# huangnengCSU/longcallR

Measured on AMD Instinct MI355X. Metric: candidate_sites_per_sec, higher is better.
Workload: dtype u8 in, u32 counts, f64 likelihoods, i64 fixed-point phase scores

## Files before the change

### include/lcr.h

```cpp
#ifndef LCR_H
#define LCR_H
#include <stddef.h>
#include <stdint.h>
#ifdef __cplusplus
extern "C" {
#endif

#define LCR_OK 0
#define LCR_E_ARG (-1)
#define LCR_E_CIGAR (-2)
#define LCR_E_DEVICE (-3)
#define LCR_E_STATE (-4)
#define LCR_E_NOMEM (-5)
#define LCR_W_HW_QUEUES 1

#define LCR_PLATFORM_HIFI 0
#define LCR_PLATFORM_ONT 1

#define LCR_MEM_HOST 0
#define LCR_MEM_DEVICE 1

typedef struct lcr_ctx lcr_ctx;


// ... 358 lines not shown
int lcr_debug_set(lcr_ctx*, const char* key, int64_t value);

enum { LCR_K_SPANS = 0 , LCR_K_PILEUP, LCR_K_CAND_FILTER, LCR_K_CAND_HIST, LCR_K_CAND_GT,
       LCR_K_FRAG_COUNT, LCR_K_FRAG_FILL, LCR_K_PHASE,
       LCR_K_BIND ,
       LCR_K_BIND_TABLE ,
       LCR_K_CAND_IMPORT , LCR_K_JUNCTIONS ,
       LCR_K_ASE , LCR_NKERNELS };
enum { LCR_K_GENES = LCR_NKERNELS ,
       LCR_K_ASE_GENES ,
       LCR_NTIMERS };
int lcr_enable_timing(lcr_ctx*, int on);
int lcr_kernel_ms(lcr_ctx*, int kernel, float* ms);
int lcr_pileup_bytes(lcr_ctx*, int64_t* bytes);
int lcr_pileup_stage_bytes(lcr_ctx*, int64_t* bytes);

int lcr_release_cached_memory(void);
int lcr_set_cache_limits(int64_t device_bytes, int64_t host_bytes);

const char* lcr_version(void);

#ifdef __cplusplus
}
#endif
#endif
```

### longcallr_amd/_lib.py

```python
import ctypes as C
import os

from . import _abi

_HERE = os.path.dirname(os.path.abspath(__file__))
SO_PATH = os.environ.get("LCR_LIB") or os.path.join(_HERE, "liblcr.so")

SYMBOLS = [
    "lcr_params_preset", "lcr_ctx_create", "lcr_ctx_destroy", "lcr_last_error", "lcr_ctx_set_stream",
    "lcr_ctx_sync", "lcr_ctx_set_lock_dir", "lcr_ctx_set_async_phase", "lcr_debug_set", "lcr_load_batch", "lcr_load_batch_async", "lcr_bind_batch",
    "lcr_host_alloc", "lcr_host_free", "lcr_host_register", "lcr_host_unregister", "lcr_pileup", "lcr_get_columns", "lcr_candidates",
    "lcr_get_candidates", "lcr_get_candidates_device", "lcr_fragments", "lcr_get_fragmat", "lcr_phase", "lcr_get_phase_result", "lcr_get_read_records_device", "lcr_collect_phase", "lcr_get_ld_blocks", "lcr_get_tie_census",
    "lcr_enable_timing", "lcr_kernel_ms", "lcr_pileup_bytes", "lcr_pileup_stage_bytes", "lcr_discover_regions", "lcr_discover_regions_truncated", "lcr_version", "lcr_release_cached_memory", "lcr_set_cache_limits",
    "lcr_bam_open", "lcr_bam_open_keep", "lcr_bam_close", "lcr_bam_last_error", "lcr_bam_refs", "lcr_bam_n_records", "lcr_bam_resident", "lcr_bam_spans", "lcr_bam_batch", "lcr_bam_write_phased", "lcr_bam_write_reads",
    "lcr_set_downsample", "lcr_set_downsample_rows", "lcr_get_downsample",
    "lcr_junctions", "lcr_get_junctions", "lcr_ase", "lcr_get_ase", "lcr_vcf_contig_alleles",
    "lcr_assign_genes", "lcr_get_read_genes", "lcr_ase_genes", "lcr_get_ase_genes",
    "lcr_junctions_genes", "lcr_get_junctions_genes", "lcr_asj_genes", "lcr_get_asj_genes",
    "lcr_load_batch_packed", "lcr_load_batch_packed_async", "lcr_unpack_bases", "lcr_unpack_ms", "lcr_bam_batch_packed",
    "lcr_set_exon_mask", "lcr_exon_mask_ms", "lcr_import_candidates", "lcr_vcf_open", "lcr_vcf_close", "lcr_vcf_last_error", "lcr_vcf_contigs", "lcr_vcf_contig",
    "lcr_haplotag", "lcr_get_haplotag_sites", "lcr_haplotag_ms", "lcr_vcf_contig_phase_sets",
    "lcr_site_counts", "lcr_get_site_counts", "lcr_site_counts_ms",
    "lcr_hap_coverage", "lcr_get_hap_coverage", "lcr_hap_coverage_ms",
    "lcr_somatic", "lcr_get_somatic", "lcr_somatic_ms",
]

_lib = None

# ... 47 lines not shown
    l.lcr_get_read_records_device.argtypes = [vp, C.POINTER(vp), C.POINTER(i32)]
    l.lcr_get_fragmat.argtypes = [vp, C.POINTER(_abi.LcrFragmat)]
    l.lcr_get_phase_result.argtypes = [vp, C.POINTER(_abi.LcrPhaseResult)]
    l.lcr_collect_phase.argtypes = [vp, C.POINTER(_abi.LcrPhaseCollected)]
    l.lcr_release_cached_memory.argtypes = []
    l.lcr_set_cache_limits.argtypes = [C.c_int64, C.c_int64]
    l.lcr_get_tie_census.argtypes = [vp, C.POINTER(C.c_uint64)]
    l.lcr_get_ld_blocks.argtypes = [vp, C.c_int32, C.POINTER(C.c_int32), C.POINTER(C.POINTER(C.c_int32)), C.POINTER(C.POINTER(C.c_int32))]
    l.lcr_discover_regions.argtypes = [vp, C.c_int32, C.c_int32, vp, vp, C.c_int64, C.POINTER(_abi.LcrRegionList)]
    l.lcr_discover_regions_truncated.argtypes = [vp, C.c_int32, C.c_int32, vp, vp, C.c_int64, C.c_int32, C.c_uint32, C.POINTER(_abi.LcrRegionList),
                                                 C.POINTER(C.c_int64)]
    l.lcr_enable_timing.argtypes = [vp, i32]
    l.lcr_kernel_ms.argtypes = [vp, i32, C.POINTER(C.c_float)]
    l.lcr_pileup_bytes.argtypes = [vp, C.POINTER(C.c_int64)]
    l.lcr_pileup_stage_bytes.argtypes = [vp, C.POINTER(C.c_int64)]
    flt = C.POINTER(_abi.LcrReadFilter)
    l.lcr_bam_open.argtypes = [C.c_char_p, C.c_int32, C.POINTER(vp)]
    l.lcr_bam_open_keep.argtypes = [C.c_char_p, C.c_int32, C.c_int64, C.POINTER(vp)]
    l.lcr_bam_close.argtypes = [vp]
    l.lcr_bam_close.restype = None
    l.lcr_bam_last_error.argtypes = [vp]
    l.lcr_bam_last_error.restype = C.c_char_p
    l.lcr_bam_refs.argtypes = [vp, C.POINTER(C.c_int32), C.POINTER(C.POINTER(C.c_char_p)), C.POINTER(C.POINTER(C.c_int64))]
    l.lcr_bam_n_records.argtypes = [vp, C.POINTER(C.c_int64)]
    l.lcr_bam_resident.argtypes = [vp, C.POINTER(C.c_int64), C.POINTER(C.c_int64)]
    l.lcr_bam_spans.argtypes = [vp, C.c_int32, flt, C.POINTER(C.c_int32), C.POINTER(C.POINTER(C.c_int32)), C.POINTER(C.POINTER(C.c_int32))]
    l.lcr_bam_batch.argtypes = [vp, C.c_int32, flt, C.c_int32, vp, vp, C.POINTER(_abi.LcrReads), C.POINTER(C.POINTER(C.c_int32)),
                                C.POINTER(C.POINTER(C.c_uint64)), C.POINTER(C.c_char_p)]
    l.lcr_bam_batch_packed.argtypes = [vp, C.c_int32, flt, C.c_int32, vp, vp, C.POINTER(_abi.LcrReadsPacked), C.POINTER(C.POINTER(C.c_int32)),
                                       C.POINTER(C.POINTER(C.c_uint64)), C.POINTER(C.c_char_p)]
# ... 44 lines not shown
```

### longcallr_amd/api.py

```python
import ctypes as C

import numpy as np

from . import _abi, _lib
from ._lib import LcrError


def _view(ptr, dtype, n):
    if n == 0 or not ptr:
        return np.zeros(0, dtype=dtype)
    buf = (C.c_char * (np.dtype(dtype).itemsize * n)).from_address(ptr)
    return np.frombuffer(buf, dtype=dtype, count=n).copy()


def _view_nocopy(ptr, dtype, n):
    if n == 0 or not ptr:
        return np.zeros(0, dtype=dtype)
    buf = (C.c_char * (np.dtype(dtype).itemsize * n)).from_address(ptr)
    return np.frombuffer(buf, dtype=dtype, count=n)


_DEBUG_ENV = {"LCR_PHASE_PROF": "phase_prof", "LCR_GRID_MIN_ENTRIES": "grid_min_entries",
              "LCR_GRID_GENERIC": "grid_generic", "LCR_GRID_SPEC_LANES": "grid_spec_lanes", "LCR_GRID_SPEC_BATCH": "grid_spec_batch", "LCR_POST_HALF": "post_half", "LCR_ENUM_FORCE_BIG": "enum_force_big",
              "LCR_ENUM_FORCE_STREAM": "enum_force_stream", "LCR_ENUM_ELIDE": "enum_elide", "LCR_HIST_TILES": "hist_tiles", "LCR_TIE_ARITH": "tie_arith", "LCR_CHAIN_TIES": "chain_ties", "LCR_K3_HITS": "k3_hits", "LCR_K3_LIST_BLOCKS": "k3_list_blocks", "LCR_FUSE_FILTER": "fuse_filter", "LCR_ASYNC_PHASE": "async_phase", "LCR_HOST_TRACE": "host_trace", "LCR_OWN_FILL": "own_fill", "LCR_REDO_LDS": "redo_lds", "LCR_SPEC_COMPACT": "spec_compact", "LCR_LEAN_PLANES": "lean_planes"}


class Engine:
    def __init__(self, device=0, params=None, timing=False):
        self.lib = _lib.load()
        h = C.c_void_p()
        rc = self.lib.lcr_ctx_create(device, C.byref(h))
        if rc != 0:
            raise LcrError("lcr_ctx_create(device=%d) failed with %d: no usable HIP device; "
                           "liblcr has no CPU fallback" % (device, rc))
        self.h = h
        self.device = device
        self.params = params if params is not None else _abi.make_params()
        self._sites = None
        self._keep = None
# ... 456 lines not shown
    def kernel_ms(self, k):
        ms = C.c_float()
        self._chk(self.lib.lcr_kernel_ms(self.h, k, C.byref(ms)), "lcr_kernel_ms")
        return float(ms.value)

    def pileup_bytes(self):
        b = C.c_int64()
        self._chk(self.lib.lcr_pileup_bytes(self.h, C.byref(b)), "lcr_pileup_bytes")
        return int(b.value)

    def pileup_stage_bytes(self):
        b = C.c_int64()
        self._chk(self.lib.lcr_pileup_stage_bytes(self.h, C.byref(b)), "lcr_pileup_stage_bytes")
        return int(b.value)


def host_register(*arrays):
    lib = _lib.load()
    done = []
    for a in arrays:
        if a is None or a.nbytes == 0:
            continue
        if lib.lcr_host_register(C.c_void_p(a.ctypes.data), a.nbytes) != 0:
            host_unregister(done)
            raise LcrError("lcr_host_register failed")
        done.append(a)
    return done


def host_unregister(arrays):
# ... 4 lines not shown
```

### longcallr_amd/csrc/k0_ops.hip

```cpp
#include <algorithm>
#include <climits>

#include "lcr_dev.h"

#ifndef K0_THREADS
#define K0_THREADS 256
#endif
#ifndef K0_OPT
#define K0_OPT 4
#endif
#ifndef K0_ABL
#define K0_ABL 0
#endif
#define K0_NW (K0_THREADS / 64)
#define K0_WIN K0_THREADS
#define K0_ACC 64
#ifndef K0_HCAP
#define K0_HCAP 160
#endif


__device__ __forceinline__ int wave_incl_max(int v) {
  v = max(v, __builtin_amdgcn_update_dpp(0, v, 0x111, 0xf, 0xf, false));
  v = max(v, __builtin_amdgcn_update_dpp(0, v, 0x112, 0xf, 0xf, false));
// ... 56 lines not shown
  uint64_t seq_off;
  int32_t reb, rel_pos;
};

__device__ __forceinline__ void wave_lds_sync() {
  __builtin_amdgcn_fence(__ATOMIC_RELEASE, "wavefront");
  __builtin_amdgcn_wave_barrier();
  __builtin_amdgcn_fence(__ATOMIC_ACQUIRE, "wavefront");
}

template <int OPT>
__global__ void __launch_bounds__(K0_THREADS)
k0_ops(BatchView b, const ReadBin* __restrict__ rbin, const int32_t* __restrict__ blk_first_read, uint64_t cig0, uint32_t n_ops,
       int ont, int D, int32_t n_tiles, int32_t* __restrict__ tile_fill, int32_t* __restrict__ tile_nchunks, int32_t* __restrict__ tile_ndiff,
       K0Ctl* __restrict__ ctl, unsigned int* __restrict__ acct, unsigned int pool_sub, unsigned long long* __restrict__ recs,
       unsigned int desc_sub, uint32_t* __restrict__ desc_tile, uint2* __restrict__ desc_val, int2* __restrict__ read_scan) {
  constexpr int OPB = OPT * K0_THREADS, WOPS = OPT * 64;
  __shared__ __attribute__((aligned(8))) uint16_t ridh[OPB];
  __shared__ K0Hdr hdr[K0_HCAP];
  __shared__ int ws_ref[K0_NW], ws_q[K0_NW], ws_rid[K0_NW];
  __shared__ int cnt[K0_WIN], cur[K0_WIN];
  __shared__ unsigned int s_base[3];
  __shared__ int runbase[OPB];
  __shared__ int s_carry[2], s_acc[2];

  const int tid = threadIdx.x, lane = tid & 63, wv = tid >> 6;
  const uint32_t j0 = blockIdx.x * (uint32_t)OPB;
  if (j0 >= n_ops) return;
  const uint32_t jend = min(j0 + (uint32_t)OPB, n_ops);
  const bool last_block = jend == n_ops;
  const uint32_t* __restrict__ cg = b.cigar + cig0;
// ... 88 lines not shown
#pragma unroll
    for (int k = 0; k < OPT; k++) {
      xr[k] += br; xq[k] += bq; rid[k] = max(rid[k], bm);
      if (mark[k] != 0) {
        if (mark[k] < K0_HCAP) { hdr[mark[k]].refbase -= xr[k]; hdr[mark[k]].qbase -= xq[k]; }
        else read_scan[r_lo + mark[k]] = make_int2(xr[k], xq[k]);
      }
    }
    if (tid == 0) { hdr[0].refbase += s_carry[0]; hdr[0].qbase += s_carry[1]; }
  }
  __syncthreads();

  if (K0_ABL == 2) { if (xr[0] + xq[1] + rid[2] == 0x7fffffff) ctl->error = 9; return; }
  int a[OPT], e[OPT], tb[OPT], kind[OPT];
  unsigned int rlo[OPT], rhi[OPT];
  unsigned int my_items = 0;
  const int win0 = hdr[0].ftile + (int)((unsigned int)max(hdr[0].rel_pos - 1, 0) / (unsigned int)LCR_TILE);
#pragma unroll
  for (int k = 0; k < OPT; k++) {
    const int p = OPT * tid + k;
    const bool act = j0 + p < jend;
    K0Hdr H;
    if (rid[k] < K0_HCAP) H = hdr[rid[k]];
    else {
      uint64_t cb; int ncig;
      H = load_hdr(r_lo + rid[k], &cb, &ncig);
      const int2 sb = read_scan[r_lo + rid[k]];
      H.refbase -= sb.x; H.qbase -= sb.y;
    }
    const int op = w[k] & 15, len = (int)(w[k] >> 4);
    const int rs = H.refbase + xr[k];
    const int qs = H.qbase + xq[k];
    const bool m = act && (op == 0 || op == 7 || op == 8), d = act && op == 2, ins = act && op == 1, isn = act && op == 3;
    int aa = max(rs, 0), ee = min(rs + len, H.vec);
    if (m) { aa = max(aa, rs + (H.qlo - qs)); ee = min(ee, rs + (H.qhi - qs)); }
    int kd = ((m || d || isn) && len > 0 && ee > aa) ? (m ? 1 : d ? 2 : 4) : 0;
    if (ins && len > 0 && rs >= 1 && rs < H.vec) { kd = 3; aa = rs - 1; ee = rs; }
    kind[k] = kd; a[k] = aa; e[k] = ee; tb[k] = H.ftile;
    if (kd == 1) {
      const unsigned long long o0 = H.seq_off + (unsigned long long)(long long)(qs - rs);
      rlo[k] = (unsigned int)o0; rhi[k] = ((unsigned int)(o0 >> 32) & 0xffu) | H.hi;
    } else {
      rlo[k] = kd == 2 ? (unsigned int)REC_KIND_D : kd == 3 ? (unsigned int)REC_KIND_I : (unsigned int)REC_KIND_N;
      rhi[k] = 0xffu;
    }
    if (kd) my_items++;
    if (act && p == H.cend - 1) {
      b.read_rend[r_lo + rid[k]] = rs + dr[k];
      if (qs + dq[k] != H.reb) atomicExch(&ctl->error, 2);
    }
    if (kd == 4) {
      const int ta = H.ftile + (int)((unsigned int)aa / (unsigned int)LCR_TILE), te = H.ftile + (int)((unsigned int)(ee - 1) / (unsigned int)LCR_TILE);
      if (te > ta + 1) { atomicAdd(&tile_ndiff[ta + 1], 1); atomicAdd(&tile_ndiff[te], -1); }
    }
  }

  if (K0_ABL == 3) { int x = 0; for (int k = 0; k < OPT; k++) x += a[k] + e[k] + tb[k] + kind[k] + (int)rlo[k] + (int)rhi[k]; if (x == 0x7fffffff) ctl->error = 9; return; }
  auto make_rec = [&](int k, int t) -> unsigned long long {
    const int c0 = (t - tb[k]) * LCR_TILE;
    const int c_lo = max(a[k], c0), c_hi = min(e[k], c0 + LCR_TILE);
    unsigned int lo = rlo[k], hi = rhi[k] | ((unsigned int)(c_lo - c0) << 8) | ((unsigned int)(c_hi - c_lo - 1) << 18);
    if (kind[k] == 1) {
      const unsigned int s = lo + (unsigned int)c_lo;
      hi = (hi & ~0xffu) | (((hi & 0xffu) + (s < lo ? 1u : 0u)) & 0xffu);
      lo = s;
    }
    return ((unsigned long long)hi << 32) | lo;
  };
  auto first_tile = [&](int k) { return tb[k] + (int)((unsigned int)a[k] / (unsigned int)LCR_TILE); };
  auto last_tile = [&](int k) { return tb[k] + (int)((unsigned int)(e[k] - 1) / (unsigned int)LCR_TILE); };
  auto next_tile = [&](int k, int t, int te) { return kind[k] == 4 ? te : t + 1; };

  int key[OPT], rank[OPT], hpos[OPT];
  bool is_last[OPT];
  {
#pragma unroll
    for (int k = 0; k < OPT; k++) {
      const int tp = kind[k] ? first_tile(k) - win0 : -1;
      key[k] = (tp >= 0 && tp < K0_WIN) ? tp : -1;
    }
    int pk = __shfl_up(key[OPT - 1], 1, 64);
    if (lane == 0) pk = -2;
    bool head[OPT];
    int hp = 0;
#pragma unroll
    for (int k = 0; k < OPT; k++) {
      head[k] = key[k] != (k == 0 ? pk : key[k - 1]);
      if (head[k]) hp = OPT * lane + k + 1;
      hpos[k] = hp;
    }
    const int ih = wave_incl_max(hp);
    int bh = __shfl_up(ih, 1, 64);
    if (lane == 0) bh = 0;
    const int nh = __shfl_down(head[0] ? 1 : 0, 1, 64);
#pragma unroll
    for (int k = 0; k < OPT; k++) {
      hpos[k] = max(hpos[k], bh) - 1;
      rank[k] = OPT * lane + k - hpos[k];
      is_last[k] = k + 1 < OPT ? head[k + 1] : (lane == 63 || nh != 0);
      if (is_last[k] && key[k] >= 0) atomicAdd(&cnt[key[k]], rank[k] + 1);
      if (kind[k]) {
        const int te = last_tile(k);
        for (int t = first_tile(k); t < te;) {
          t = next_tile(k, t, te);
          const int wi = t - win0;
          if (wi >= 0 && wi < K0_WIN) atomicAdd(&cnt[wi], 1);
        }
      }
    }
  }
  __syncthreads();

  if (K0_ABL == 4) { int x = 0; for (int k = 0; k < OPT; k++) x += rank[k] + hpos[k] + (is_last[k] ? 1 : 0); if (x == 0x7fffffff) ctl->error = 9; return; }
  unsigned int my_recs = 0;
  const unsigned int shard = blockIdx.x % K0_ACC;
  {
// ... 21 lines not shown
    if (c > 0 && s_base[2]) {
      const int tile = win0 + tid;
      const unsigned int di = s_base[1] + (unsigned int)dbefore + (unsigned int)__popcll(nzb & ((1ull << lane) - 1ull));
      desc_tile[di] = (uint32_t)tile; desc_val[di] = make_uint2(s_base[0] + (unsigned int)(before + ic - c16), (unsigned int)c);
      atomicAdd(&tile_fill[tile], c);
      atomicAdd(&tile_nchunks[tile], c16 >> 4);
    }
  }
  const unsigned int blk_at = s_base[0];
  const bool blk_fits = s_base[2] != 0;

  auto put = [&](int slot, unsigned long long rec) { if (blk_fits) recs[blk_at + (unsigned int)slot] = rec; };
  int* rbw = runbase + wv * WOPS;
#pragma unroll
  for (int k = 0; k < OPT; k++)
    if (is_last[k] && key[k] >= 0) rbw[hpos[k]] = atomicAdd(&cur[key[k]], rank[k] + 1);
  wave_lds_sync();
  bool overflow = false;
#pragma unroll
  for (int k = 0; k < OPT; k++) {
    if (key[k] >= 0) put(rbw[hpos[k]] + rank[k], make_rec(k, first_tile(k)));
    else if (kind[k]) overflow = true;
    if (kind[k]) {
      const int te = last_tile(k);
      for (int t = first_tile(k); t < te;) {
        t = next_tile(k, t, te);
        const int wi = t - win0;
        if (wi >= 0 && wi < K0_WIN) put(atomicAdd(&cur[wi], 1), make_rec(k, t));
        else overflow = true;
      }
    }
  }
  if (overflow) {
#pragma unroll
    for (int k = 0; k < OPT; k++) {
      if (!kind[k]) continue;
      const int te = last_tile(k);
      for (int t = first_tile(k);; t = next_tile(k, t, te)) {
        if (t - win0 < 0 || t - win0 >= K0_WIN) {
          unsigned int* sh = acct + 32 * shard;
          const unsigned int at = atomicAdd(&sh[2], 1u), di = atomicAdd(&sh[3], 1u);
          if (at >= pool_sub || di >= desc_sub) atomicExch(&ctl->error, 3);
          else {
            recs[shard * pool_sub + at] = make_rec(k, t);
            desc_tile[shard * desc_sub + di] = (uint32_t)t; desc_val[shard * desc_sub + di] = make_uint2(shard * pool_sub + at, 1u);
            atomicAdd(&tile_fill[t], 1);
            atomicAdd(&tile_nchunks[t], 1);
          }
          my_recs++;
        }
        if (t >= te) break;
// ... 34 lines not shown
    const int ne = (int)((d.y + 15u) >> 4);
    uint2* dst = sorted + chunk_off[t] + atomicAdd(&cursor[t], ne);
    for (int e = 0; e < ne; e++) dst[e] = make_uint2(d.x + 16u * (unsigned int)e, min(16u, d.y - 16u * (unsigned int)e));
  }
}
void launch_k0_desc_bin(const K0Ctl* ctl, const unsigned int* acct, unsigned int desc_sub, const uint32_t* desc_tile, const void* desc_val,
                        const int32_t* chunk_off, int32_t* cursor, void* sorted, int32_t n_blocks_hint, hipStream_t s) {
  const int per = std::max(1, std::min((n_blocks_hint + K0_ACC - 1) / K0_ACC, 32));
  hipLaunchKernelGGL(k0_desc_bin, dim3(per * K0_ACC), dim3(LCR_BLOCK), 0, s, ctl, acct, desc_sub, desc_tile, (const uint2*)desc_val,
                     chunk_off, cursor, (uint2*)sorted);
}

void launch_k0_ops(const BatchView& b, const ReadBin* rb, const int32_t* blk_first_read, uint64_t cig0, uint32_t n_ops, int ont, int D,
                   int32_t n_tiles, int32_t* tile_fill, int32_t* tile_nchunks, int32_t* tile_ndiff, K0Ctl* ctl, unsigned int* acct,
                   unsigned int pool_sub, unsigned long long* recs, unsigned int desc_sub, uint32_t* desc_tile, void* desc_val, void* read_scan,
                   hipStream_t s) {
  if (b.n_reads == 0) return;
  if (n_ops == 0) { hipLaunchKernelGGL(k0_empty_reads, dim3((b.n_reads + LCR_BLOCK - 1) / LCR_BLOCK), dim3(LCR_BLOCK), 0, s, b, rb, ctl); return; }
  const int opb = launch_k0_opb();
  hipLaunchKernelGGL(k0_ops<K0_OPT>, dim3((n_ops + opb - 1) / opb), dim3(K0_THREADS), 0, s, b, rb, blk_first_read, cig0, n_ops, ont, D, n_tiles,
                     tile_fill, tile_nchunks, tile_ndiff, ctl, acct, pool_sub, recs, desc_sub, desc_tile, (uint2*)desc_val, (int2*)read_scan);
}
```

### longcallr_amd/csrc/k1_pileup.hip

```cpp
#include <algorithm>
#include <climits>

#include "lcr_dev.h"
#include "k2_eval.h"

#ifdef LCR_K1_ABLATE
#define K1_ABL LCR_K1_ABLATE
#else
#define K1_ABL 0
#endif
#ifndef K1_THREADS
#define K1_THREADS LCR_TILE
#endif
#define K1_WAVES (K1_THREADS / 64)
#define K1_CPT (LCR_TILE / K1_THREADS)
#define K1_RPB 2
#define K1_PMAP (8 * K1_THREADS)
#ifndef K1_NT_STORES
#define K1_NT_STORES 0
#endif
#ifndef K1_PIF
#define K1_PIF 4
#endif

// ... 244 lines not shown
  unsigned long long rec_nx[K1_RPB];
  int has_nx = load_recs(tid * K1_RPB, rec_nx);
  for (int rbase = 0; rbase < n_slots && K1_ABL != 3; rbase += K1_RPB * K1_THREADS) {
    unsigned long long rec_cur[K1_RPB];
#pragma unroll
    for (int x = 0; x < K1_RPB; x++) rec_cur[x] = rec_nx[x];
    const int has_cur = has_nx;
    has_nx = load_recs(rbase + K1_RPB * K1_THREADS + tid * K1_RPB, rec_nx);
    int npc[K1_RPB], nsum = 0;
#pragma unroll
    for (int x = 0; x < K1_RPB; x++) {
      const int slot = tid * K1_RPB + x;
      const unsigned long long rec = rec_cur[x];
      const bool hasrec = (has_cur >> x) & 1;
      const unsigned long long off = rec & REC_OFF_MASK;
      const int col0 = (int)((rec >> 40) & 1023u), len = (int)((rec >> 50) & 1023u) + 1;
      int npieces = 0;
      if (hasrec) {
        if (off == REC_KIND_D) {
          atomicAdd(&pl[P_DIFF_D * TSTRIDE + col0], 1u);
          atomicAdd(&pl[P_DIFF_D * TSTRIDE + col0 + len], 0xFFFFFFFFu);
        } else if (off == REC_KIND_I) {
          atomicAdd(&pl[P_NI * TSTRIDE + col0], 1u);
        } else if (off == REC_KIND_N) {
          atomicAdd(&pl[P_DIFF_N * TSTRIDE + col0], 1u);
          atomicAdd(&pl[P_DIFF_N * TSTRIDE + col0 + len], 0xFFFFFFFFu);
        } else {
          const int strand = (int)((rec >> 60) & 1u), tscls = (int)((rec >> 61) & 3u);
          uint32_t* dp = pl + (strand ? P_DIFF_DEPTH_R : P_DIFF_DEPTH_F) * TSTRIDE;
          atomicAdd(&dp[col0], 1u);
          atomicAdd(&dp[col0 + len], 0xFFFFFFFFu);
          if (tscls) {
            uint32_t* tp = pl + (tscls == 2 ? P_DIFF_TS1 : P_DIFF_TS0) * TSTRIDE;
            atomicAdd(&tp[col0], 1u);
            atomicAdd(&tp[col0 + len], 0xFFFFFFFFu);
          }
          npieces = (len + 15) >> 4;
        }
      }
      rec_s[slot] = rec;
      npc[x] = K1_ABL == 1 ? 0 : npieces;
      nsum += npc[x];
    }
    int run = block_incl_scan(nsum, wsum) - nsum;
    int P = 0;
#pragma unroll
    for (int i = 0; i < K1_WAVES; i++) P += wsum[i];
    const int pstride = (P + K1_PMAP - 1) / K1_PMAP;
    if (tid == 0) pstart[0] = 0;
#pragma unroll
    for (int x = 0; x < K1_RPB; x++) {
// ... 3 lines not shown
      if (pstride == 1) for (int q = first; q < run; q++) pown[q] = (uint16_t)(tid * K1_RPB + x);
      else if (pstride > 1) for (int k = (first + pstride - 1) / pstride; k * pstride < run; k++) pown[k] = (uint16_t)(tid * K1_RPB + x);
    }
    __syncthreads();
    struct Piece { uint4 v; int colA, k_lo, k_hi, strand; bool ok; };
    auto fetch = [&](int p) -> Piece {
      Piece q;
      q.ok = p < P;
      if (!q.ok) { q.v = make_uint4(0, 0, 0, 0); q.colA = 0; q.k_lo = q.k_hi = 0; q.strand = 0; return q; }
      int lo;
      if (pstride == 1) lo = pown[p];
      else { lo = pown[p / pstride]; while (pstart[lo + 1] <= p) lo++; }
      const unsigned long long rc = rec_s[lo];
      const uint32_t rhi = (uint32_t)(rc >> 32);
      const long long soff = (long long)(rc & REC_OFF_MASK);
      const int scol = (int)((rhi >> 8) & 1023u), slen = (int)((rhi >> 18) & 1023u) + 1;
      q.strand = (int)((rhi >> 28) & 1u);
      const int d16 = 16 * (p - pstart[lo]);
      const long long A = soff + d16;
      q.k_lo = 0; q.k_hi = min(16, slen - d16);
      q.colA = scol + d16;
      if (A + 16 <= b.n_bases) q.v = *reinterpret_cast<const uint4*>(b.bases + A);
      else {
        uint32_t t[4] = {0, 0, 0, 0};
        for (int x = 0; x < 16; x++)
          if (A + x < b.n_bases) t[x >> 2] |= (uint32_t)b.bases[A + x] << (8 * (x & 3));
        q.v = make_uint4(t[0], t[1], t[2], t[3]);
      }
      return q;
    };
    auto tally = [&](const Piece& q) {
// ... 567 lines not shown
```

### longcallr_amd/csrc/k2_candidates.hip

```cpp
#include "lcr_dev.h"
#include "k2_eval.h"

#define SCAN_ITEMS 4
#define SCAN_TILE (LCR_BLOCK * SCAN_ITEMS)

__device__ __forceinline__ int wave_incl_scan_i(int v, int lane) {
#pragma unroll
  for (int d = 1; d < 64; d <<= 1) {
    int t = __shfl_up(v, d, 64);
    if (lane >= d) v += t;
  }
  return v;
}
__device__ __forceinline__ long long wave_incl_scan_ll(long long v, int lane) {
#pragma unroll
  for (int d = 1; d < 64; d <<= 1) {
    long long t = __shfl_up(v, d, 64);
    if (lane >= d) v += t;
  }
  return v;
}

template <typename OutT>
__global__ void __launch_bounds__(LCR_BLOCK) scan_phase1(const int32_t* __restrict__ in, OutT* __restrict__ out, int32_t n,
// ... 295 lines not shown
    for (int i = tid; i < pc; i += HT_BLOCK) slot_of[sv[s0 + p0 + i].col - tc0] = (uint16_t)i;
    __syncthreads();
    const int c_lo = sv[s0 + p0].col - tc0, c_hi = sv[s0 + p0 + pc - 1].col - tc0;
    auto fetch = [&](int j) -> unsigned long long {
      if (j >= j_hi) return ~0ull;
      const uint2 en = ents[e0 + (j >> 4)];
      return ((unsigned int)j & 15u) < en.y ? recs[en.x + ((unsigned int)j & 15u)] : ~0ull;
    };
    unsigned long long nx = fetch(j_lo + grp), nx2 = fetch(j_lo + grp + HT_BLOCK / HT_LANES);
    for (int j = j_lo + grp; j < j_hi; j += HT_BLOCK / HT_LANES) {
      const unsigned long long rec = nx;
      nx = nx2;
      nx2 = fetch(j + 2 * (HT_BLOCK / HT_LANES));
      const unsigned long long off = rec & REC_OFF_MASK;
      const bool live = off < REC_KIND_N;
      const int col0 = (int)((rec >> 40) & 1023u), len = (int)((rec >> 50) & 1023u) + 1;
      const int d_lo = max(0, c_lo - col0), d_hi = live ? min(len - 1, c_hi - col0) : -1;
      auto tally = [&](int dd, bool in, uint32_t base, uint32_t qual) {
        const uint32_t slot = slot_of[min(col0 + max(dd, 0), LCR_TILE - 1)];
        const uint32_t u = (base & 0xDFu) - 65u;
        const bool acgt = u < 20u && ((0x80045u >> u) & 1u);
        const uint32_t k = ((base & 0xDFu) >> 1) & 3u, bi = k ^ (k >> 1);
        const uint32_t q = min(qual, 30u);
        const uint32_t idx = slot * 124u + bi * 31u + q;
        if (in && acgt && slot != 0xFFFFu) atomicAdd(&hp[idx >> 1], 1u << (16 * (idx & 1u)));
      };
      for (int d0 = d_lo + 4 * ln; d0 <= d_hi; d0 += 4 * HT_LANES) {
        const unsigned long long at = off + (unsigned long long)d0;
        uint32_t bw, qw;
        if (at + 4 <= (unsigned long long)b.n_bases) {
          bw = *reinterpret_cast<const uint32_t*>(b.bases + at); qw = *reinterpret_cast<const uint32_t*>(b.quals + at);
// ... 267 lines not shown
```

### longcallr_amd/csrc/lcr_api.hip

```cpp
#include <chrono>
#include <cmath>
#include <cstdlib>
#include <map>
#include <mutex>

#include "lcr_ctx.h"

namespace {
struct BlockCache {
  std::mutex mu;
  std::multimap<size_t, void*> blocks[2][16];
  size_t held[2][16] = {};
  size_t limit[2] = {(size_t)24 << 30, (size_t)2 << 30};
};
BlockCache& block_cache() { static BlockCache* c = new BlockCache(); return *c; }
}
void* lcr_cache_take(int host, size_t want, size_t* cap) {
  int dev = 0;
  if (hipGetDevice(&dev) != hipSuccess || dev < 0 || dev >= 16) return nullptr;
  BlockCache& bc = block_cache();
  std::lock_guard<std::mutex> g(bc.mu);
  auto& m = bc.blocks[host ? 1 : 0][dev];
  auto it = m.lower_bound(want);
  if (it == m.end() || it->first > 2 * want + (1u << 20)) return nullptr;
// ... 203 lines not shown

int lcr_pileup_bytes(lcr_ctx* c, int64_t* bytes) {
  if (!c || !bytes) return LCR_E_ARG;
  int64_t staged = 0;
  const int rc = pile_staged_bytes(c, &staged);
  *bytes = c->pileup_bytes + staged;
  return rc;
}

int lcr_pileup_stage_bytes(lcr_ctx* c, int64_t* bytes) {
  if (!c || !bytes) return LCR_E_ARG;
  int64_t staged = 0;
  const int rc = pile_staged_bytes(c, &staged);
  *bytes = c->stage_bytes + staged;
  return rc;
}

int lcr_phase(lcr_ctx* c, const lcr_params* p) {
  if (!c || !p) return LCR_E_ARG;
  if (c->stage < ST_FRAGGED) { c->err = "lcr_phase before lcr_fragments"; return LCR_E_STATE; }
  if (c->cand_used) { c->err = "lcr_phase after lcr_phase: the phase stage has rewritten the candidate records; run the candidate stage again"; return LCR_E_STATE; }
  if (p->ld_weight_threshold != 1) { c->err = "ld_weight_threshold must be 1: SNPFrag::phase is only ever called with 1 (thread.rs:166)"; return LCR_E_ARG; }
  const bool ds_on = c->ds_rows_set || c->ds_depth > 0;
  if (ds_on && !(p->read_assign_cutoff > 0.0)) { c->err = "down-sampling needs read_assign_cutoff > 0: the last read assignment must not depend on the sign of an unsampled row's haplotag"; return LCR_E_ARG; }
  HIPCHK(c, hipSetDevice(c->device));
  { int rc = frag_settle(c); if (rc) return rc; }
  PhaseInputs in;
  in.ds_depth = c->ds_depth; in.ds_seed = c->ds_seed; in.ds_rows = c->ds_rows_set ? c->ds_rows.data() : nullptr;
  c->ds_rows_set = false;
  in.n_regions = c->bv.n_regions; in.n_rows = c->n_rows; in.nnz = c->nnz;
// ... 230 lines not shown
        HIPCHK(c, hipMemcpyAsync(host.data(), buf.p, 4 * N, hipMemcpyDeviceToHost, c->stream));
        HIPCHK(c, hipStreamSynchronize(c->stream));
        if (host != want) { c->err = "fill_selftest: a fill kernel wrote other bytes than asked (offset " + std::to_string(off) + ", length " + std::to_string(len) + ")"; return LCR_E_DEVICE; }
      }
  }
  else if (k == "chain_ties") d.chain_ties = value != 0;
  else if (k == "redo_lds") d.redo_lds = (int)std::max<int64_t>(0, std::min<int64_t>(value, 128 * 1024));
  else if (k == "tie_arith") d.tie_arith = (int)std::max<int64_t>(0, std::min<int64_t>(value, 3));
  else if (k == "timing_mask") c->timing_mask = (uint32_t)value;
  else if (k == "hist_tiles") c->dbg_hist_tiles = value > 0 ? 1 : value < 0 ? -1 : 0;
  else if (k == "k3_hits") c->dbg_k3_hits = value != 0;
  else if (k == "k3_list_blocks") c->dbg_k3_list_blocks = (int)std::max<int64_t>(0, std::min<int64_t>(value, 65536));
  else if (k == "fuse_filter") c->dbg_fuse_filter = value != 0;
  else if (k == "spec_compact") c->dbg_spec_compact = value != 0;
  else if (k == "lean_planes") c->dbg_lean_planes = value != 0;
  else if (k == "poison_planes") c->dbg_poison_planes = value != 0;
  else if (k == "grid_spec_batch") d.spec_batch = (int)value;
  else if (k == "grid_spec_lanes") d.spec_lanes = (int)std::max<int64_t>(1, std::min<int64_t>(value, 16));
  else { c->err = "lcr_debug_set: unknown key " + k; return LCR_E_ARG; }
  return LCR_OK;
}

int lcr_get_ld_blocks(lcr_ctx* c, int32_t region, int32_t* n_blocks, const int32_t** block_off, const int32_t** snp_idx) {
  if (!c || !n_blocks || !block_off || !snp_idx) return LCR_E_ARG;
  if (c->stage < ST_PHASED) { c->err = "lcr_get_ld_blocks before lcr_phase"; return LCR_E_STATE; }
  if (region < 0 || region >= c->bv.n_regions) { c->err = "lcr_get_ld_blocks: no such region"; return LCR_E_ARG; }
  { int rc = phase_settle(c); if (rc) return rc; }
  PhaseInputs in;
  in.n_regions = c->bv.n_regions;
  in.cand_region_off = c->h_cand_off.data();
// ... 16 lines not shown
```

### longcallr_amd/csrc/lcr_ctx.h

```cpp
#pragma once
#include <algorithm>
#include <cstring>

#include "lcr_dev.h"
#include "lcr_phase_host.h"

enum Stage { ST_NONE, ST_LOADED, ST_PILED, ST_CALLED, ST_FRAGGED, ST_PHASED };

struct AnnotationCopy { DevBuf span_s, span_e, exon_off, exon_s, exon_e; };

struct SlotTable {
  int32_t n_slots = 0;
  DevBuf tbl_key, tbl_cnt, flag, koff;
  DevBuf ck, cc, cp;
  DevBuf off;
};

struct GeneJunctions {
  bool valid = false;
  bool timed = false;
  int32_t n = 0, ng = 0;
  AnnotationCopy ann;
  DevBuf part, nocc, part_off, occ_off, cnt, pair_off, read_pair, row_slot, pregion, pgene, prow0, prows, pocc, tsz, tbl_off, rows, keys, jpair;
  SlotTable t;
// ... 35 lines not shown
  struct UploadSlot { DevBuf buf[16]; DevBuf seq4, pack_off;
                      hipEvent_t ev = nullptr; bool filled = false; lcr_reads rd{}; lcr_regions rg{}; } up[2];
  hipStream_t up_stream = nullptr;
  int bound_slot = -1;
  bool bound_host = false;
  DevBuf in_seq4, in_pack_off, unpacked;
  HostBuf h_unpack_bad;
  hipEvent_t ev_unpack_t[2] = {};
  bool unpack_timed = false;
  DevBuf scan_tmp, read_region, read_bin, read_rend, tile_region, tile_col0, first_tile, k0_tile_fill, k0_items, tile_nbase, tile_order;
  DevBuf desc_tile, desc_val, chunks, chunk_off;
  DevBuf blk_first_read, read_scan, cig_compact, cig_off_new, cig_new_off32;
  uint64_t cig0 = 0;
  uint32_t n_ops = 0;
  int64_t n_items = 0;

  bool planes_dense = false;
  bool planes_tallied = false;
  int dbg_poison_planes = 0;
  int dbg_lean_planes = 1;
  DevBuf planes;
  bool sv_staged = false;
  int32_t sv_stage_cap = 0;
  int64_t sv_stage_n = -1;
  DevBuf sv_stage, sv_stage_key;
  DevParams dp{};
  int32_t pile_platform = -1; uint32_t pile_dist_to_end = 0;
  float sor_thr = -1.f;
  HostBuf h_planes;
  HostBuf h_nnz;
// ... 226 lines not shown
```

### longcallr_amd/csrc/lcr_dev.h

```cpp
#pragma once
#include <hip/hip_runtime.h>
#include <climits>
#include <cstddef>
#include <stdint.h>

#include <string>
#include <vector>

#include "../../include/lcr.h"

#ifndef LCR_TILE
#define LCR_TILE 256
#endif
#define LCR_BLOCK 256
#define LCR_WAVE 64

struct BatchView {
  int32_t n_reads, n_regions;
  int64_t n_bases;
  const int32_t* pos;
  const int32_t* seq_len;
  const int32_t* lead;
  const int32_t* trail;
  const uint8_t* flags;
// ... 26 lines not shown
  int32_t flags, pad_;
  int64_t pad2_;
};
static_assert(sizeof(ReadBin) == 64, "ReadBin must be 64 bytes");

struct DevParams {
  int32_t ont;
  int32_t dist_to_end, polya_len;
  uint32_t min_baseq, min_depth, max_depth, min_qual, low_cnt_cut, min_linkers;
  int32_t use_strand_bias;
  float min_af, min_af_intron, low_frac_cut;
  float sor_threshold;
  int32_t dbg;
};

#define REC_OFF_MASK 0xFFFFFFFFFFull
#define REC_KIND_D 0xFFFFFFFFFFull
#define REC_KIND_I 0xFFFFFFFFFEull
#define REC_KIND_N 0xFFFFFFFFFDull

struct Survivor {
  int64_t gcol;
  int32_t region;
  int32_t col;
  uint8_t ref_base, allele1, allele2, n_alt;
  uint32_t cnt1, cnt2, depth;
  uint32_t ts_fwd, ts_rev;
  float af1, af2;
};

// ... 83 lines not shown
void launch_k0_bind_a(const int64_t* start0, const int32_t* len, const int64_t* col_off, const int32_t* read_begin, int32_t ng,
                      int32_t* first_tile, int64_t* h_start0, int32_t* h_len, int64_t* h_col_off, int32_t* h_read_begin,
                      const uint64_t* cig_off, const uint32_t* n_cig, int32_t nr, int64_t n_cigar, int32_t* out, hipStream_t s);
void launch_k0_bind_b(const BatchView& b, ReadBin* rbin, int32_t* order_flag, int32_t* read_region, int32_t n_tiles, int32_t* tile_region,
                      int32_t* tile_col0, uint64_t cig0, int32_t opb, int32_t n_blocks, int32_t* blk_first_read, hipStream_t s);
void launch_k0_unpack(int32_t nr, const int32_t* seq_len, const uint64_t* seq_off, const uint64_t* pack_off, const uint8_t* seq4, int64_t n_pack,
                      uint8_t* out, int64_t n_bases, int32_t* bad , hipStream_t s);
void launch_k0_cig_check(const uint64_t* cig_off, const uint32_t* n_cig, int32_t nr, int64_t n_cigar, int32_t* out, hipStream_t s);
void launch_k0_cig_compact(const uint32_t* cigar, const uint64_t* cig_off, const uint32_t* n_cig, const int32_t* new_off, int32_t nr,
                           uint32_t* out, uint64_t* out_off, hipStream_t s);
int launch_k0_opb();
void launch_k0_block_reads(const ReadBin* rbin, int32_t nr, uint64_t cig0, int32_t opb, int32_t n_blocks, int32_t* blk_first_read, hipStream_t s);
void launch_k0_ops(const BatchView& b, const ReadBin* rb, const int32_t* blk_first_read, uint64_t cig0, uint32_t n_ops, int ont, int D,
                   int32_t n_tiles, int32_t* tile_fill, int32_t* tile_nchunks, int32_t* tile_ndiff, K0Ctl* ctl, unsigned int* acct ,
                   unsigned int pool_sub , unsigned long long* recs, unsigned int desc_sub, uint32_t* desc_tile, void* desc_val ,
                   void* read_scan , hipStream_t s);
int launch_k0_acct_words();
int launch_k0_acct_slots();
void launch_k0_desc_bin(const K0Ctl* ctl, const unsigned int* acct, unsigned int desc_sub, const uint32_t* desc_tile, const void* desc_val,
                        const int32_t* chunk_off, int32_t* cursor , void* sorted , int32_t n_blocks_hint,
                        hipStream_t s);
size_t launch_k1_tiles_tmp_words(int32_t n_tiles);
struct PileScratch {
  size_t ctl;
  size_t ndiff;
  size_t nch;
  size_t cur;
  size_t acct;
  size_t tmp;
  size_t words;
};
// ... 342 lines not shown
```

### longcallr_amd/csrc/lcr_pileup.hip

```cpp
#include "lcr_ctx.h"

namespace {

struct PilePools {
  int32_t n_blocks = 0;
  size_t pool_cap64 = 0, desc_cap64 = 0;
  size_t n_shards = 0;
  unsigned int pool_sub = 0, desc_sub = 0;
};

PilePools pile_size_pools(const lcr_ctx* c) {
  PilePools P;
  const int opb = launch_k0_opb();
  P.n_blocks = (int32_t)(((uint64_t)c->n_ops + opb - 1) / opb);
  P.desc_cap64 = (size_t)P.n_blocks * 128 + (size_t)c->bv.n_reads / 4 + 1024;
  P.pool_cap64 = (size_t)c->n_ops + (size_t)c->n_ops / 2 + (size_t)c->bv.n_reads + (size_t)c->n_bases / LCR_TILE + 8 * P.desc_cap64 + 1024;
  return P;
}

int pile_reserve_pools(lcr_ctx* c, PilePools& P) {
  const size_t nsh = P.n_shards = (size_t)launch_k0_acct_slots();
  const size_t pool_sub64 = (P.pool_cap64 + nsh - 1) / nsh + 256, desc_sub64 = (P.desc_cap64 + nsh - 1) / nsh + 64;
  if (pool_sub64 * nsh > 0xFFFFFFF0ull || desc_sub64 * nsh > 0x7FFFFFF0ull) { c->err = "batch too large for the 32-bit record pool: split it"; return LCR_E_ARG; }
  P.pool_sub = (unsigned int)pool_sub64; P.desc_sub = (unsigned int)desc_sub64;
// ... 11 lines not shown
  HIPCHK(c, c->tile_order.reserve(std::max(nt, 1) * 4));
  HIPCHK(c, c->tile_nbase.reserve(std::max(nt, 1) * 4));
  HIPCHK(c, c->chunk_off.reserve(((size_t)nt + 2) * 4));
  HIPCHK(c, c->read_scan.reserve(std::max<size_t>(c->bv.n_reads, 1) * 8));
  HIPCHK(c, c->h_stage[0].reserve(64));
  return LCR_OK;
}

int pile_queue_k0(lcr_ctx* c, const PileScratch& L, const PilePools& P, bool& gated) {
  int32_t* const fill = c->k0_tile_fill.as<int32_t>();
  HIPCHK(c, lcr_fill_async(fill, 0, L.words * 4, c->stream));
  if (!gated) { HIPCHK(c, c->phase.gate_stream(c->stream)); gated = true; }
  Timer t(c, LCR_K_SPANS);
  launch_k0_ops(c->bv, c->read_bin.as<ReadBin>(), c->blk_first_read.as<int32_t>(), c->cig0, c->n_ops, c->dp.ont, c->dp.dist_to_end, c->n_tiles,
                fill, fill + L.nch, fill + L.ndiff, reinterpret_cast<K0Ctl*>(fill + L.ctl), (unsigned int*)(fill + L.acct), P.pool_sub, c->k0_items.as<unsigned long long>(),
                P.desc_sub, c->desc_tile.as<uint32_t>(), c->desc_val.p, c->read_scan.p, c->stream);
  return LCR_OK;
}

int pile_queue_tally(lcr_ctx* c, const PileScratch& L, const PilePools& P, bool fuse, bool lean) {
  BatchView& b = c->bv;
  const int nt = c->n_tiles;
  int32_t* const fill = c->k0_tile_fill.as<int32_t>();
  K0Ctl* const d_ctl = reinterpret_cast<K0Ctl*>(fill + L.ctl);
  { Timer t(c, LCR_K_PILEUP);
    if (nt > 0) {
      K0Ctl* h_ctl_dev = nullptr;
      HIPCHK(c, c->h_stage[0].dev(&h_ctl_dev));
      launch_k1_tiles_a(nt, fill, fill + L.ndiff, fill + L.nch, fill + L.tmp, (unsigned int*)(fill + L.acct), launch_k0_acct_slots(),
                        d_ctl, h_ctl_dev, c->tile_region.as<int32_t>(), c->tile_col0.as<int32_t>(), b.len, c->stream);
    } else HIPCHK(c, hipMemcpyAsync(c->h_stage[0].p, d_ctl, sizeof(K0Ctl), hipMemcpyDeviceToHost, c->stream));
// ... 138 lines not shown
```

Baseline: 6.853 billion.

## Fold short indels into preceding match records to shrink pileup record stream

```diff
diff --git a/include/lcr.h b/include/lcr.h
--- a/include/lcr.h
+++ b/include/lcr.h
@@ -396,6 +396,7 @@
 int lcr_kernel_ms(lcr_ctx*, int kernel, float* ms);
 int lcr_pileup_bytes(lcr_ctx*, int64_t* bytes);
 int lcr_pileup_stage_bytes(lcr_ctx*, int64_t* bytes);
+int lcr_pileup_records(lcr_ctx*, int64_t* n);
 
 int lcr_release_cached_memory(void);
 int lcr_set_cache_limits(int64_t device_bytes, int64_t host_bytes);
diff --git a/longcallr_amd/_lib.py b/longcallr_amd/_lib.py
--- a/longcallr_amd/_lib.py
+++ b/longcallr_amd/_lib.py
@@ -11,7 +11,7 @@
     "lcr_ctx_sync", "lcr_ctx_set_lock_dir", "lcr_ctx_set_async_phase", "lcr_debug_set", "lcr_load_batch", "lcr_load_batch_async", "lcr_bind_batch",
     "lcr_host_alloc", "lcr_host_free", "lcr_host_register", "lcr_host_unregister", "lcr_pileup", "lcr_get_columns", "lcr_candidates",
     "lcr_get_candidates", "lcr_get_candidates_device", "lcr_fragments", "lcr_get_fragmat", "lcr_phase", "lcr_get_phase_result", "lcr_get_read_records_device", "lcr_collect_phase", "lcr_get_ld_blocks", "lcr_get_tie_census",
-    "lcr_enable_timing", "lcr_kernel_ms", "lcr_pileup_bytes", "lcr_pileup_stage_bytes", "lcr_discover_regions", "lcr_discover_regions_truncated", "lcr_version", "lcr_release_cached_memory", "lcr_set_cache_limits",
+    "lcr_enable_timing", "lcr_kernel_ms", "lcr_pileup_bytes", "lcr_pileup_stage_bytes", "lcr_pileup_records", "lcr_discover_regions", "lcr_discover_regions_truncated", "lcr_version", "lcr_release_cached_memory", "lcr_set_cache_limits",
     "lcr_bam_open", "lcr_bam_open_keep", "lcr_bam_close", "lcr_bam_last_error", "lcr_bam_refs", "lcr_bam_n_records", "lcr_bam_resident", "lcr_bam_spans", "lcr_bam_batch", "lcr_bam_write_phased", "lcr_bam_write_reads",
     "lcr_set_downsample", "lcr_set_downsample_rows", "lcr_get_downsample",
     "lcr_junctions", "lcr_get_junctions", "lcr_ase", "lcr_get_ase", "lcr_vcf_contig_alleles",
@@ -89,6 +89,8 @@
     l.lcr_kernel_ms.argtypes = [vp, i32, C.POINTER(C.c_float)]
     l.lcr_pileup_bytes.argtypes = [vp, C.POINTER(C.c_int64)]
     l.lcr_pileup_stage_bytes.argtypes = [vp, C.POINTER(C.c_int64)]
+    if hasattr(l, "lcr_pileup_records"):
+        l.lcr_pileup_records.argtypes = [vp, C.POINTER(C.c_int64)]
     flt = C.POINTER(_abi.LcrReadFilter)
     l.lcr_bam_open.argtypes = [C.c_char_p, C.c_int32, C.POINTER(vp)]
     l.lcr_bam_open_keep.argtypes = [C.c_char_p, C.c_int32, C.c_int64, C.POINTER(vp)]
diff --git a/longcallr_amd/api.py b/longcallr_amd/api.py
--- a/longcallr_amd/api.py
+++ b/longcallr_amd/api.py
@@ -22,7 +22,7 @@
 
 _DEBUG_ENV = {"LCR_PHASE_PROF": "phase_prof", "LCR_GRID_MIN_ENTRIES": "grid_min_entries",
               "LCR_GRID_GENERIC": "grid_generic", "LCR_GRID_SPEC_LANES": "grid_spec_lanes", "LCR_GRID_SPEC_BATCH": "grid_spec_batch", "LCR_POST_HALF": "post_half", "LCR_ENUM_FORCE_BIG": "enum_force_big",
-              "LCR_ENUM_FORCE_STREAM": "enum_force_stream", "LCR_ENUM_ELIDE": "enum_elide", "LCR_HIST_TILES": "hist_tiles", "LCR_TIE_ARITH": "tie_arith", "LCR_CHAIN_TIES": "chain_ties", "LCR_K3_HITS": "k3_hits", "LCR_K3_LIST_BLOCKS": "k3_list_blocks", "LCR_FUSE_FILTER": "fuse_filter", "LCR_ASYNC_PHASE": "async_phase", "LCR_HOST_TRACE": "host_trace", "LCR_OWN_FILL": "own_fill", "LCR_REDO_LDS": "redo_lds", "LCR_SPEC_COMPACT": "spec_compact", "LCR_LEAN_PLANES": "lean_planes"}
+              "LCR_ENUM_FORCE_STREAM": "enum_force_stream", "LCR_ENUM_ELIDE": "enum_elide", "LCR_HIST_TILES": "hist_tiles", "LCR_TIE_ARITH": "tie_arith", "LCR_CHAIN_TIES": "chain_ties", "LCR_K3_HITS": "k3_hits", "LCR_K3_LIST_BLOCKS": "k3_list_blocks", "LCR_FUSE_FILTER": "fuse_filter", "LCR_ASYNC_PHASE": "async_phase", "LCR_HOST_TRACE": "host_trace", "LCR_OWN_FILL": "own_fill", "LCR_REDO_LDS": "redo_lds", "LCR_SPEC_COMPACT": "spec_compact", "LCR_LEAN_PLANES": "lean_planes", "LCR_FOLD_INDELS": "fold_indels"}
 
 
 class Engine:
@@ -509,6 +509,11 @@
         self._chk(self.lib.lcr_pileup_stage_bytes(self.h, C.byref(b)), "lcr_pileup_stage_bytes")
         return int(b.value)
 
+    def pileup_records(self):
+        n = C.c_int64()
+        self._chk(self.lib.lcr_pileup_records(self.h, C.byref(n)), "lcr_pileup_records")
+        return int(n.value)
+
 
 def host_register(*arrays):
     lib = _lib.load()
diff --git a/longcallr_amd/csrc/k0_ops.hip b/longcallr_amd/csrc/k0_ops.hip
--- a/longcallr_amd/csrc/k0_ops.hip
+++ b/longcallr_amd/csrc/k0_ops.hip
@@ -94,7 +94,7 @@
 k0_ops(BatchView b, const ReadBin* __restrict__ rbin, const int32_t* __restrict__ blk_first_read, uint64_t cig0, uint32_t n_ops,
        int ont, int D, int32_t n_tiles, int32_t* __restrict__ tile_fill, int32_t* __restrict__ tile_nchunks, int32_t* __restrict__ tile_ndiff,
        K0Ctl* __restrict__ ctl, unsigned int* __restrict__ acct, unsigned int pool_sub, unsigned long long* __restrict__ recs,
-       unsigned int desc_sub, uint32_t* __restrict__ desc_tile, uint2* __restrict__ desc_val, int2* __restrict__ read_scan) {
+       unsigned int desc_sub, uint32_t* __restrict__ desc_tile, uint2* __restrict__ desc_val, int2* __restrict__ read_scan, int fold) {
   constexpr int OPB = OPT * K0_THREADS, WOPS = OPT * 64;
   __shared__ __attribute__((aligned(8))) uint16_t ridh[OPB];
   __shared__ K0Hdr hdr[K0_HCAP];
@@ -213,6 +213,7 @@
   if (K0_ABL == 2) { if (xr[0] + xq[1] + rid[2] == 0x7fffffff) ctl->error = 9; return; }
   int a[OPT], e[OPT], tb[OPT], kind[OPT];
   unsigned int rlo[OPT], rhi[OPT];
+  bool whole[OPT];
   unsigned int my_items = 0;
   const int win0 = hdr[0].ftile + (int)((unsigned int)max(hdr[0].rel_pos - 1, 0) / (unsigned int)LCR_TILE);
 #pragma unroll
@@ -236,6 +237,7 @@
     int kd = ((m || d || isn) && len > 0 && ee > aa) ? (m ? 1 : d ? 2 : 4) : 0;
     if (ins && len > 0 && rs >= 1 && rs < H.vec) { kd = 3; aa = rs - 1; ee = rs; }
     kind[k] = kd; a[k] = aa; e[k] = ee; tb[k] = H.ftile;
+    whole[k] = ee == rs + len;
     if (kd == 1) {
       const unsigned long long o0 = H.seq_off + (unsigned long long)(long long)(qs - rs);
       rlo[k] = (unsigned int)o0; rhi[k] = ((unsigned int)(o0 >> 32) & 0xffu) | H.hi;
@@ -254,11 +256,33 @@
     }
   }
 
+  unsigned int rfold[OPT];
+  bool emits[OPT];
+  {
+    unsigned int fb[OPT];
+    static_assert((LCR_TILE & (LCR_TILE - 1)) == 0, "two columns lie in one tile iff they differ below LCR_TILE");
+    bool pmt = __shfl_up(kind[OPT - 1] == 1 && whole[OPT - 1] ? 1 : 0, 1, 64) != 0 && lane != 0 && fold;
+#pragma unroll
+    for (int k = 0; k < OPT; k++) {
+      const int len = e[k] - a[k];
+      const bool d_ok = kind[k] == 2 && whole[k] && len <= REC_FOLD_DMAX && (unsigned int)((e[k] - 1) ^ (a[k] - 1)) < (unsigned int)LCR_TILE;
+      const bool f = pmt && mark[k] == 0 && (kind[k] == 3 || d_ok);
+      const unsigned int dbits = ((unsigned int)len * ((1u << REC_FOLD_D0_HI) | (1u << (REC_FOLD_D1_HI - 2)))) & ((3u << REC_FOLD_D0_HI) | (3u << REC_FOLD_D1_HI));
+      fb[k] = !f ? 0u : kind[k] == 3 ? REC_FOLD_I_HI : dbits;
+      emits[k] = kind[k] != 0 && !f;
+      pmt = kind[k] == 1 && whole[k] && fold;
+    }
+    const unsigned int nf = (unsigned int)__shfl_down((int)fb[0], 1, 64);
+#pragma unroll
+    for (int k = 0; k < OPT; k++) rfold[k] = k + 1 < OPT ? fb[k + 1] : (lane == 63 ? 0u : nf);
+  }
+
   if (K0_ABL == 3) { int x = 0; for (int k = 0; k < OPT; k++) x += a[k] + e[k] + tb[k] + kind[k] + (int)rlo[k] + (int)rhi[k]; if (x == 0x7fffffff) ctl->error = 9; return; }
   auto make_rec = [&](int k, int t) -> unsigned long long {
     const int c0 = (t - tb[k]) * LCR_TILE;
     const int c_lo = max(a[k], c0), c_hi = min(e[k], c0 + LCR_TILE);
     unsigned int lo = rlo[k], hi = rhi[k] | ((unsigned int)(c_lo - c0) << 8) | ((unsigned int)(c_hi - c_lo - 1) << 18);
+    if (c_hi == e[k]) hi |= rfold[k];
     if (kind[k] == 1) {
       const unsigned int s = lo + (unsigned int)c_lo;
       hi = (hi & ~0xffu) | (((hi & 0xffu) + (s < lo ? 1u : 0u)) & 0xffu);
@@ -271,21 +295,26 @@
   auto next_tile = [&](int k, int t, int te) { return kind[k] == 4 ? te : t + 1; };
 
   int key[OPT], rank[OPT], hpos[OPT];
-  bool is_last[OPT];
+  bool is_last[OPT], draws[OPT];
   {
+    int nslot[OPT], tn = 0;
 #pragma unroll
     for (int k = 0; k < OPT; k++) {
       const int tp = kind[k] ? first_tile(k) - win0 : -1;
       key[k] = (tp >= 0 && tp < K0_WIN) ? tp : -1;
-    }
+      draws[k] = emits[k] && key[k] >= 0;
+      nslot[k] = tn; tn += draws[k] ? 1 : 0;
+    }
+    const int bn = wave_incl_scan(tn) - tn;
     int pk = __shfl_up(key[OPT - 1], 1, 64);
     if (lane == 0) pk = -2;
     bool head[OPT];
     int hp = 0;
 #pragma unroll
     for (int k = 0; k < OPT; k++) {
+      nslot[k] += bn;
       head[k] = key[k] != (k == 0 ? pk : key[k - 1]);
-      if (head[k]) hp = OPT * lane + k + 1;
+      if (head[k]) hp = nslot[k] + 1;
       hpos[k] = hp;
     }
     const int ih = wave_incl_max(hp);
@@ -295,10 +324,10 @@
 #pragma unroll
     for (int k = 0; k < OPT; k++) {
       hpos[k] = max(hpos[k], bh) - 1;
-      rank[k] = OPT * lane + k - hpos[k];
-      is_last[k] = k + 1 < OPT ? head[k + 1] : (lane == 63 || nh != 0);
-      if (is_last[k] && key[k] >= 0) atomicAdd(&cnt[key[k]], rank[k] + 1);
-      if (kind[k]) {
+      rank[k] = nslot[k] - hpos[k];
+      is_last[k] = (k + 1 < OPT ? head[k + 1] : (lane == 63 || nh != 0)) && key[k] >= 0 && rank[k] + (draws[k] ? 1 : 0) > 0;
+      if (is_last[k]) atomicAdd(&cnt[key[k]], rank[k] + (draws[k] ? 1 : 0));
+      if (emits[k]) {
         const int te = last_tile(k);
         for (int t = first_tile(k); t < te;) {
           t = next_tile(k, t, te);
@@ -350,14 +379,14 @@
   int* rbw = runbase + wv * WOPS;
 #pragma unroll
   for (int k = 0; k < OPT; k++)
-    if (is_last[k] && key[k] >= 0) rbw[hpos[k]] = atomicAdd(&cur[key[k]], rank[k] + 1);
+    if (is_last[k]) rbw[hpos[k]] = atomicAdd(&cur[key[k]], rank[k] + (draws[k] ? 1 : 0));
   wave_lds_sync();
   bool overflow = false;
 #pragma unroll
   for (int k = 0; k < OPT; k++) {
-    if (key[k] >= 0) put(rbw[hpos[k]] + rank[k], make_rec(k, first_tile(k)));
-    else if (kind[k]) overflow = true;
-    if (kind[k]) {
+    if (draws[k]) put(rbw[hpos[k]] + rank[k], make_rec(k, first_tile(k)));
+    else if (emits[k]) overflow = true;
+    if (emits[k]) {
       const int te = last_tile(k);
       for (int t = first_tile(k); t < te;) {
         t = next_tile(k, t, te);
@@ -370,7 +399,7 @@
   if (overflow) {
 #pragma unroll
     for (int k = 0; k < OPT; k++) {
-      if (!kind[k]) continue;
+      if (!emits[k]) continue;
       const int te = last_tile(k);
       for (int t = first_tile(k);; t = next_tile(k, t, te)) {
         if (t - win0 < 0 || t - win0 >= K0_WIN) {
@@ -435,10 +464,10 @@
 void launch_k0_ops(const BatchView& b, const ReadBin* rb, const int32_t* blk_first_read, uint64_t cig0, uint32_t n_ops, int ont, int D,
                    int32_t n_tiles, int32_t* tile_fill, int32_t* tile_nchunks, int32_t* tile_ndiff, K0Ctl* ctl, unsigned int* acct,
                    unsigned int pool_sub, unsigned long long* recs, unsigned int desc_sub, uint32_t* desc_tile, void* desc_val, void* read_scan,
-                   hipStream_t s) {
+                   int fold, hipStream_t s) {
   if (b.n_reads == 0) return;
   if (n_ops == 0) { hipLaunchKernelGGL(k0_empty_reads, dim3((b.n_reads + LCR_BLOCK - 1) / LCR_BLOCK), dim3(LCR_BLOCK), 0, s, b, rb, ctl); return; }
   const int opb = launch_k0_opb();
   hipLaunchKernelGGL(k0_ops<K0_OPT>, dim3((n_ops + opb - 1) / opb), dim3(K0_THREADS), 0, s, b, rb, blk_first_read, cig0, n_ops, ont, D, n_tiles,
-                     tile_fill, tile_nchunks, tile_ndiff, ctl, acct, pool_sub, recs, desc_sub, desc_tile, (uint2*)desc_val, (int2*)read_scan);
-}
+                     tile_fill, tile_nchunks, tile_ndiff, ctl, acct, pool_sub, recs, desc_sub, desc_tile, (uint2*)desc_val, (int2*)read_scan, fold);
+}
diff --git a/longcallr_amd/csrc/k1_pileup.hip b/longcallr_amd/csrc/k1_pileup.hip
--- a/longcallr_amd/csrc/k1_pileup.hip
+++ b/longcallr_amd/csrc/k1_pileup.hip
@@ -282,7 +282,7 @@
       const unsigned long long rec = rec_cur[x];
       const bool hasrec = (has_cur >> x) & 1;
       const unsigned long long off = rec & REC_OFF_MASK;
-      const int col0 = (int)((rec >> 40) & 1023u), len = (int)((rec >> 50) & 1023u) + 1;
+      const int col0 = (int)((rec >> 40) & REC_COL_MASK), len = (int)((rec >> 50) & REC_COL_MASK) + 1;
       int npieces = 0;
       if (hasrec) {
         if (off == REC_KIND_D) {
@@ -303,6 +303,11 @@
             atomicAdd(&tp[col0], 1u);
             atomicAdd(&tp[col0 + len], 0xFFFFFFFFu);
           }
+          if (REC_FOLD_I(rec)) atomicAdd(&pl[P_NI * TSTRIDE + col0 + len - 1], 1u);
+          if (const int dl = REC_FOLD_D(rec)) {
+            atomicAdd(&pl[P_DIFF_D * TSTRIDE + col0 + len], 1u);
+            atomicAdd(&pl[P_DIFF_D * TSTRIDE + col0 + len + dl], 0xFFFFFFFFu);
+          }
           npieces = (len + 15) >> 4;
         }
       }
@@ -336,7 +341,7 @@
       const unsigned long long rc = rec_s[lo];
       const uint32_t rhi = (uint32_t)(rc >> 32);
       const long long soff = (long long)(rc & REC_OFF_MASK);
-      const int scol = (int)((rhi >> 8) & 1023u), slen = (int)((rhi >> 18) & 1023u) + 1;
+      const int scol = (int)((rhi >> 8) & REC_COL_MASK), slen = (int)((rhi >> 18) & REC_COL_MASK) + 1;
       q.strand = (int)((rhi >> 28) & 1u);
       const int d16 = 16 * (p - pstart[lo]);
       const long long A = soff + d16;
diff --git a/longcallr_amd/csrc/k2_candidates.hip b/longcallr_amd/csrc/k2_candidates.hip
--- a/longcallr_amd/csrc/k2_candidates.hip
+++ b/longcallr_amd/csrc/k2_candidates.hip
@@ -333,7 +333,7 @@
       nx2 = fetch(j + 2 * (HT_BLOCK / HT_LANES));
       const unsigned long long off = rec & REC_OFF_MASK;
       const bool live = off < REC_KIND_N;
-      const int col0 = (int)((rec >> 40) & 1023u), len = (int)((rec >> 50) & 1023u) + 1;
+      const int col0 = (int)((rec >> 40) & REC_COL_MASK), len = (int)((rec >> 50) & REC_COL_MASK) + 1;
       const int d_lo = max(0, c_lo - col0), d_hi = live ? min(len - 1, c_hi - col0) : -1;
       auto tally = [&](int dd, bool in, uint32_t base, uint32_t qual) {
         const uint32_t slot = slot_of[min(col0 + max(dd, 0), LCR_TILE - 1)];
diff --git a/longcallr_amd/csrc/lcr_api.hip b/longcallr_amd/csrc/lcr_api.hip
--- a/longcallr_amd/csrc/lcr_api.hip
+++ b/longcallr_amd/csrc/lcr_api.hip
@@ -241,6 +241,13 @@
   const int rc = pile_staged_bytes(c, &staged);
   *bytes = c->stage_bytes + staged;
   return rc;
+}
+
+int lcr_pileup_records(lcr_ctx* c, int64_t* n) {
+  if (!c || !n) return LCR_E_ARG;
+  if (c->stage < ST_PILED) { c->err = "lcr_pileup_records before lcr_pileup"; return LCR_E_STATE; }
+  *n = c->n_items;
+  return LCR_OK;
 }
 
 int lcr_phase(lcr_ctx* c, const lcr_params* p) {
@@ -501,6 +508,7 @@
   else if (k == "fuse_filter") c->dbg_fuse_filter = value != 0;
   else if (k == "spec_compact") c->dbg_spec_compact = value != 0;
   else if (k == "lean_planes") c->dbg_lean_planes = value != 0;
+  else if (k == "fold_indels") c->dbg_fold_indels = value != 0;
   else if (k == "poison_planes") c->dbg_poison_planes = value != 0;
   else if (k == "grid_spec_batch") d.spec_batch = (int)value;
   else if (k == "grid_spec_lanes") d.spec_lanes = (int)std::max<int64_t>(1, std::min<int64_t>(value, 16));
diff --git a/longcallr_amd/csrc/lcr_ctx.h b/longcallr_amd/csrc/lcr_ctx.h
--- a/longcallr_amd/csrc/lcr_ctx.h
+++ b/longcallr_amd/csrc/lcr_ctx.h
@@ -73,6 +73,7 @@
   uint64_t cig0 = 0;
   uint32_t n_ops = 0;
   int64_t n_items = 0;
+  int dbg_fold_indels = 1;
 
   bool planes_dense = false;
   bool planes_tallied = false;
diff --git a/longcallr_amd/csrc/lcr_dev.h b/longcallr_amd/csrc/lcr_dev.h
--- a/longcallr_amd/csrc/lcr_dev.h
+++ b/longcallr_amd/csrc/lcr_dev.h
@@ -64,6 +64,15 @@
   int32_t dbg;
 };
 
+#define REC_COL_BITS 8
+#define REC_COL_MASK ((1u << REC_COL_BITS) - 1u)
+static_assert(LCR_TILE <= (1 << REC_COL_BITS), "a record's tile column and length - 1 take REC_COL_BITS bits each: the fold bits lie behind them");
+#define REC_FOLD_DMAX 15
+#define REC_FOLD_I_HI (1u << 31)
+#define REC_FOLD_D0_HI 16
+#define REC_FOLD_D1_HI 26
+#define REC_FOLD_I(rec) ((int)((rec) >> 63))
+#define REC_FOLD_D(rec) ((int)((((rec) >> 48) & 3u) | ((((rec) >> 58) & 3u) << 2)))
 #define REC_OFF_MASK 0xFFFFFFFFFFull
 #define REC_KIND_D 0xFFFFFFFFFFull
 #define REC_KIND_I 0xFFFFFFFFFEull
@@ -177,7 +186,7 @@
 void launch_k0_ops(const BatchView& b, const ReadBin* rb, const int32_t* blk_first_read, uint64_t cig0, uint32_t n_ops, int ont, int D,
                    int32_t n_tiles, int32_t* tile_fill, int32_t* tile_nchunks, int32_t* tile_ndiff, K0Ctl* ctl, unsigned int* acct ,
                    unsigned int pool_sub , unsigned long long* recs, unsigned int desc_sub, uint32_t* desc_tile, void* desc_val ,
-                   void* read_scan , hipStream_t s);
+                   void* read_scan , int fold , hipStream_t s);
 int launch_k0_acct_words();
 int launch_k0_acct_slots();
 void launch_k0_desc_bin(const K0Ctl* ctl, const unsigned int* acct, unsigned int desc_sub, const uint32_t* desc_tile, const void* desc_val,
diff --git a/longcallr_amd/csrc/lcr_pileup.hip b/longcallr_amd/csrc/lcr_pileup.hip
--- a/longcallr_amd/csrc/lcr_pileup.hip
+++ b/longcallr_amd/csrc/lcr_pileup.hip
@@ -49,7 +49,7 @@
   Timer t(c, LCR_K_SPANS);
   launch_k0_ops(c->bv, c->read_bin.as<ReadBin>(), c->blk_first_read.as<int32_t>(), c->cig0, c->n_ops, c->dp.ont, c->dp.dist_to_end, c->n_tiles,
                 fill, fill + L.nch, fill + L.ndiff, reinterpret_cast<K0Ctl*>(fill + L.ctl), (unsigned int*)(fill + L.acct), P.pool_sub, c->k0_items.as<unsigned long long>(),
-                P.desc_sub, c->desc_tile.as<uint32_t>(), c->desc_val.p, c->read_scan.p, c->stream);
+                P.desc_sub, c->desc_tile.as<uint32_t>(), c->desc_val.p, c->read_scan.p, c->dbg_fold_indels, c->stream);
   return LCR_OK;
 }
 
```

Result: faster. 6.941 billion (median of 6 runs) (+1.3%).
